# jmduarte/gnn-fpga

Measured on AMD Instinct MI355X. Metric: edges/sec (EdgeNet+NodeNet fwd) on 100k-edge TrackML graphs; % HBM roofline, higher is better.
Workload: dtype f32; 1 GPU; c3 synthetic TrackML ACTS graphs: 256 graphs/launch/GPU x (10k hits, 100k segments), F=3, D=8, 3 MP iterations + final edge pass, index form resident in HBM; graphs_per_gpu=256, hits_per_graph=10000, segments_per_graph=100000

## Files before the change

### gnn-fpga_amd/csrc/sell_pipeline.hip

```cpp
#include "common.h"

#include <cstdlib>
#include <type_traits>
#include <utility>

namespace {
using namespace gnn;

constexpr int SLICE = 16;
constexpr int DESC = 8;

template <int F, int D>
struct TL {
    static constexpr int d4 = D / 4, C = F + D;
    static constexpr int a4(int x) { return (x + 3) & ~3; }
    static constexpr int o_w2 = 0;
    static constexpr int o_in = a4(o_w2 + d4);
    static constexpr int in_sz = d4 + F * d4;
    static constexpr int o_4 = a4(o_in + in_sz);
    static constexpr int w4_sz = d4 + D * d4;
    static constexpr int o_m = a4(o_4 + w4_sz);
    static constexpr int m_sz = d4 + C * d4;
    static constexpr int m_st = a4(m_sz);
    static constexpr int o_b2 = o_m + 5 * m_st;
// ... 1430 lines not shown
    __device__ __forceinline__ void second(float *f) const { f[0] = bf_lo(w.z); f[1] = bf_hi(w.z); f[2] = bf_lo(w.w); f[3] = bf_hi(w.w); }
};
template <> struct PieceW<1> {
    unsigned w;
    __device__ __forceinline__ void load(const void *a) { w = *reinterpret_cast<const unsigned *>(a); }
    __device__ __forceinline__ void first(float *f) const { f[0] = bf_lo(w); }
    __device__ __forceinline__ void second(float *f) const { f[0] = bf_hi(w); }
};
template <> struct PieceW<2> {
    uint2 w;
    __device__ __forceinline__ void load(const void *a) { w = *reinterpret_cast<const uint2 *>(a); }
    __device__ __forceinline__ void first(float *f) const { f[0] = bf_lo(w.x); f[1] = bf_hi(w.x); }
    __device__ __forceinline__ void second(float *f) const { f[0] = bf_lo(w.y); f[1] = bf_hi(w.y); }
};
template <int DL> struct PieceX;
template <> struct PieceX<4> {
    float4 a, b;
    __device__ __forceinline__ void load(const void *p)
    {
        a = reinterpret_cast<const float4 *>(p)[0];
        b = reinterpret_cast<const float4 *>(p)[16];
    }
    __device__ __forceinline__ void first(float *f) const { f[0] = a.x; f[1] = a.y; f[2] = a.z; f[3] = a.w; }
    __device__ __forceinline__ void second(float *f) const { f[0] = b.x; f[1] = b.y; f[2] = b.z; f[3] = b.w; }
};
template <> struct PieceX<1> {
    float2 a;
    __device__ __forceinline__ void load(const void *p) { a = *reinterpret_cast<const float2 *>(p); }
    __device__ __forceinline__ void first(float *f) const { f[0] = a.x; }
    __device__ __forceinline__ void second(float *f) const { f[0] = a.y; }
};
template <> struct PieceX<2> {
    float4 a;
    __device__ __forceinline__ void load(const void *p) { a = *reinterpret_cast<const float4 *>(p); }
    __device__ __forceinline__ void first(float *f) const { f[0] = a.x; f[1] = a.y; }
    __device__ __forceinline__ void second(float *f) const { f[0] = a.z; f[1] = a.w; }
};

template <int D, bool EX = false>
struct RecW {
    static constexpr int DL = D / 16;
    static constexpr unsigned row_bytes = (EX ? 8 : 4) * D;
    static constexpr unsigned piece_bytes = row_halves<D, EX>() ? 4 * DL : (EX ? 8 : 4) * DL;
    std::conditional_t<EX, PieceX<DL>, PieceW<DL>> r[4];
    __device__ __forceinline__ void read(int cur, const void *__restrict__ REC, unsigned lane_off)
    {
        const int nb[4] = {quad_bcast_i<0>(cur), quad_bcast_i<1>(cur), quad_bcast_i<2>(cur), quad_bcast_i<3>(cur)};
#pragma unroll
        for (int j = 0; j < 4; ++j)
            r[j].load(reinterpret_cast<const char *>(REC) + ((unsigned)nb[j] * row_bytes + lane_off));
    }
};

template <int D, bool XP, bool EX = false>
__device__ __forceinline__ void score_w(const RecW<D, EX> &g, const float *own, const float *w2, float b2, int p,
                                        float *acc)
{
    constexpr int DL = D / 16;
    static_assert(DL == 1 || DL % 2 == 0, "one dimension per lane, or dimension pairs");
    const f2_t one2 = {1.0f, 1.0f};
    float part[4];
#pragma unroll
    for (int j = 0; j < 4; ++j) {
        float P[DL];
        g.r[j].first(P);
        if constexpr (DL == 1) {
            const float a = XP ? fmaf(P[0], own[0], 1.0f) : __builtin_amdgcn_exp2f(P[0] + own[0]) + 1.0f;
            part[j] = w2[0] * __builtin_amdgcn_rcpf(a);
        } else {
            f2_t s2 = {0.0f, 0.0f};
#pragma unroll
            for (int i = 0; i + 1 < DL; i += 2) {
                const f2_t pj = {P[i], P[i + 1]}, o2 = {own[i], own[i + 1]};
                f2_t a;
                if constexpr (XP) {
                    a = pj * o2 + one2;
                } else {
                    const f2_t z = pj + o2;
                    a = f2_t{__builtin_amdgcn_exp2f(z.x), __builtin_amdgcn_exp2f(z.y)} + one2;
                }
                const f2_t r = {__builtin_amdgcn_rcpf(a.x), __builtin_amdgcn_rcpf(a.y)};
                s2 = f2_t{w2[i], w2[i + 1]} * r + s2;
            }
            part[j] = s2.x + s2.y;
        }
    }
    const int q = p & 3;
    const bool odd = q & 1, hi = q & 2;
    const float s0 = odd ? part[0] : part[1], s1 = odd ? part[2] : part[3];
    const float k0 = odd ? part[1] : part[0], k1 = odd ? part[3] : part[2];
    const float t0 = k0 + dpp<0xB1>(s0), t1 = k1 + dpp<0xB1>(s1);
    const float give = hi ? t0 : t1, keep = hi ? t1 : t0;
    float mine = keep + dpp<0x4E>(give);
    mine += dpp_row<0x124>(mine);
    mine += dpp_row<0x128>(mine);
    const float e = r_f(mine + b2);
    const float e4[4] = {quad_bcast_f<0>(e), quad_bcast_f<1>(e), quad_bcast_f<2>(e), quad_bcast_f<3>(e)};
#pragma unroll
    for (int j = 0; j < 4; ++j) {
        float R[DL];
        g.r[j].second(R);
        if constexpr (DL == 1) {
            acc[0] = fmaf(R[0], e4[j], acc[0]);
        } else {
            const f2_t e2 = {e4[j], e4[j]};
#pragma unroll
            for (int i = 0; i + 1 < DL; i += 2) {
                const f2_t a2 = f2_t{R[i], R[i + 1]} * e2 + f2_t{acc[i], acc[i + 1]};
                acc[i] = a2.x;
                acc[i + 1] = a2.y;
            }
        }
    }
}

template <int D, bool XP, bool EX = false>
__device__ __forceinline__ void sweep_w(const int32_t *__restrict__ lst, int i16, int len, int null_idx,
                                        const void *__restrict__ REC, int p, const float *own, const float *w2,
                                        float b2, float *acc)
{
    if (len <= 0) return;
    constexpr int DL = D / 16;
    const int ng = (len + 3) >> 2;
    const unsigned lane_off = RecW<D, EX>::piece_bytes * (unsigned)p;
    const unsigned st_off = (unsigned)((SLICE * (p & 3) + i16) * 4);
    auto index_of = [&](int c) {
        const int cur = *reinterpret_cast<const int32_t *>(reinterpret_cast<const char *>(lst) +
                                                             ((unsigned)(c * 4 * SLICE * 4) + st_off));
        return 4 * c + (p & 3) < len ? cur : null_idx;
    };
    RecW<D, EX> a, b;
    int ia = index_of(0), ib = ng > 1 ? index_of(1) : 0;
    a.read(ia, REC, lane_off);
    for (int c = 0; c < ng; c += 2) {
        if (c + 1 < ng) b.read(ib, REC, lane_off);
        if (c + 2 < ng) ia = index_of(c + 2);
        score_w<D, XP, EX>(a, own, w2, b2, p, acc);
        if (c + 1 < ng) {
            if (c + 2 < ng) a.read(ia, REC, lane_off);
            if (c + 3 < ng) ib = index_of(c + 3);
            score_w<D, XP, EX>(b, own, w2, b2, p, acc);
        }
    }
}

template <int D, bool EX>
__device__ __forceinline__ void load_own_w(const unsigned *__restrict__ REC, int64_t n, int p, float *out)
{
    constexpr int DL = D / 16;
    if constexpr (row_halves<D, EX>()) {
        load_vec<DL>(reinterpret_cast<const float *>(REC) + n * 2 * D + DL * p, out);
    } else {
        constexpr int WPR = EX ? 2 * D : D, WPL = EX ? 2 * DL : DL;
        std::conditional_t<EX, PieceX<DL>, PieceW<DL>> w;
        w.load(REC + n * WPR + WPL * p);
        w.first(out);
    }
}

template <int F, int D, bool LAST, bool XP, bool EX = false>
__global__ __launch_bounds__(1024, (D == 16 ? 8 : 4)) void k_iter_w(
    const float *__restrict__ X, const float *__restrict__ table, const unsigned *__restrict__ t16,
    const int32_t *__restrict__ tiles, const int32_t *__restrict__ in_off, const int32_t *__restrict__ in_nbr,
    const int32_t *__restrict__ out_off, const int32_t *__restrict__ out_nbr, const unsigned *__restrict__ PR,
    const unsigned *__restrict__ QS, float *__restrict__ U, float *__restrict__ PRn, float *__restrict__ QSn,
    float *__restrict__ Pc, float *__restrict__ Qc, int64_t n_pad, int tiles_per_xcd, int n_tiles, int wmax)
{
    using L = TL<F, D>;
    using B = std::conditional_t<EX, BX<F, D>, BL<F, D>>;
    static_assert(D % 16 == 0, "16 lanes x D / 16 dims per hit, matrix-core tail");
    extern __shared__ __attribute__((aligned(16))) float smem[];
    int *grp = reinterpret_cast<int *>(smem + B::template lds_words<LAST>() + (EX ? 12 : 8) * 16 * B::tr_stride);
    unsigned *tb = reinterpret_cast<unsigned *>(smem);
    {
        constexpr int n1 = B::NT1 * B::KS1 * (EX ? 64 : 256), nm = B::template tm_words<LAST>();
        for (int i = threadIdx.x; i < n1; i += 1024) tb[i] = t16[B::o_t4 + i];
        for (int i = threadIdx.x; i < nm; i += 1024) tb[n1 + i] = t16[(LAST ? B::o_tml : B::o_tmn) + i];
        for (int i = threadIdx.x; i < D; i += 1024) tb[n1 + nm + i] = t16[B::o_b4 + i];
        for (int i = threadIdx.x; i < (LAST ? 2 : 5) * D; i += 1024)
            tb[n1 + nm + D + i] = t16[(LAST ? B::o_bml : B::o_bmn) + i];
    }
    const int lane = threadIdx.x & 63, wv = threadIdx.x >> 6;
    const int hs = lane >> 4, p = lane & 15;
    const int team = wv >> 2, mem = wv & 3;
    float *scratch = smem + B::template lds_words<LAST>();
    constexpr int DL = D / 16;
    float w2[DL];
#pragma unroll
    for (int i = 0; i < DL; ++i) w2[i] = table[(p >> 2) * L::stride + L::o_w2 + DL * (p & 3) + i];
    const float b2 = table[L::o_b2];
    const int xcd = blockIdx.x & 7, local = blockIdx.x >> 3, per_xcd = gridDim.x >> 3;
    const int t_begin = xcd * tiles_per_xcd;
    const int t_end = t_begin + tiles_per_xcd < n_tiles ? t_begin + tiles_per_xcd : n_tiles;
    __syncthreads();
    if (t_begin >= t_end) return;
    int buf = 0, rot = 0;
    for (int t = t_begin; t < t_end;) {
        if (wv == 0) {
            const int tt = t + lane;
            const bool in = tt < t_end;
            const int32_t *d = tiles + (int64_t)(in ? tt : t) * DESC;
            const int s1 = d[1];
            int ilo = in && d[3] > 0 ? d[2] : 0x7FFFFFFF, ihi = in && d[3] > 0 ? d[2] + d[3] : -1;
            int olo = in && d[5] > 0 ? d[4] : 0x7FFFFFFF, ohi = in && d[5] > 0 ? d[4] + d[5] : -1;
#pragma unroll
            for (int o = 1; o < 64; o <<= 1) {
                const int a = __shfl_up(ilo, o, 64), b = __shfl_up(ihi, o, 64);
                const int c = __shfl_up(olo, o, 64), e = __shfl_up(ohi, o, 64);
                if (lane >= o) {
                    ilo = a < ilo ? a : ilo; ihi = b > ihi ? b : ihi;
                    olo = c < olo ? c : olo; ohi = e > ohi ? e : ohi;
                }
            }
            const bool ok = in && (lane == 0 || ((int64_t)ihi - ilo <= wmax && (int64_t)ohi - olo <= wmax));
            const unsigned long long m = ~__ballot(ok);
            const int cnt = m ? __builtin_ctzll(m) : 64;
            const int send = __shfl(s1, cnt - 1, 64);
            if (lane == 0) { grp[0] = d[0]; grp[1] = send; grp[2] = t + cnt; }
        }
        __syncthreads();
        const int sg0 = grp[0], sg1 = grp[1];
        t = grp[2];
        __syncthreads();
        const int nq = (sg1 - sg0 + 3) >> 2;
        const int q0 = (((local - rot) % per_xcd) + per_xcd) % per_xcd;
        rot = (rot + nq) % per_xcd;
        const int x0 = sg0;
        constexpr bool SPLIT = EX && D >= 64;
        for (int q = q0; SPLIT && x0 + 4 * q < sg1; q += per_xcd) {
            const int sl = x0 + 4 * q + team;
            if (sl < sg0 || sl >= sg1) continue;
            const int ib = __builtin_amdgcn_readfirstlane(in_off[sl]);
            const int il = (__builtin_amdgcn_readfirstlane(in_off[sl + 1]) - ib) >> 4;
            if (il <= 0) continue;
            const int i16 = 4 * mem + hs;
            const int64_t n = (int64_t)sl * SLICE + i16;
            float acc[DL], ownQ[DL];
            load_vec<DL>(U + n * D + DL * p, acc);
            load_own_w<D, EX>(QS, n, p, ownQ);
#ifndef GNN_ABLATE_W_SWEEP
            sweep_w<D, XP, EX>(in_nbr + ib, i16, il, (int)n_pad, PR, p, ownQ, w2, b2, acc);
#endif
            store_vec<DL>(U + n * D + DL * p, acc);
        }
        for (int q = q0; x0 + 4 * q < sg1; q += per_xcd, buf ^= 1) {
            const int sl = x0 + 4 * q + team;
            const bool on = sl >= sg0 && sl < sg1;
            float *tr = scratch + (buf * 4 + team) * 16 * B::tr_stride;
            if (on) {
                const int ob = __builtin_amdgcn_readfirstlane(out_off[sl]);
                const int ol = (__builtin_amdgcn_readfirstlane(out_off[sl + 1]) - ob) >> 4;
                const int i16 = 4 * mem + hs;
                const int64_t n = (int64_t)sl * SLICE + i16;
                float acc[DL], ownP[DL];
                load_vec<DL>(U + n * D + DL * p, acc);
                if constexpr (!SPLIT) {
                    const int ib = __builtin_amdgcn_readfirstlane(in_off[sl]);
                    const int il = (__builtin_amdgcn_readfirstlane(in_off[sl + 1]) - ib) >> 4;
                    float ownQ[DL];
                    load_own_w<D, EX>(QS, n, p, ownQ);
                    load_own_w<D, EX>(PR, n, p, ownP);
                    sweep_w<D, XP, EX>(in_nbr + ib, i16, il, (int)n_pad, PR, p, ownQ, w2, b2, acc);
                } else {
                    load_own_w<D, EX>(PR, n, p, ownP);
                }
#ifndef GNN_ABLATE_W_SWEEP
                sweep_w<D, XP, EX>(out_nbr + ob, i16, ol, (int)n_pad, QS, p, ownP, w2, b2, acc);
#endif
#pragma unroll
                for (int i = 0; i < DL; ++i) acc[i] = tanh_f(acc[i]);
                store_vec<DL>(tr + i16 * B::tr_stride + DL * p, acc);
                if (p < F) tr[i16 * B::tr_stride + D + p] = X[n * F + p];
            }
            __syncthreads();
            if constexpr (EX) {
                float *th = scratch + (8 + team) * 16 * B::tr_stride;
#ifndef GNN_ABLATE_W_TAIL
                if (on) mfma_hidden_x<F, D, LAST>(smem, tr, th, lane, mem);
#endif
                __syncthreads();
#ifndef GNN_ABLATE_W_TAIL
                if (on)
                    mfma_tail_scratch_x<F, D, LAST, XP>(smem, tr, th, lane, (int64_t)sl * SLICE, PRn, QSn, U, Pc, Qc, mem, 4);
#endif
            } else if (on) {
                mfma_tail_scratch<F, D, LAST, XP>(tb, tr, lane, (int64_t)sl * SLICE, PRn, QSn, U, Pc, Qc, mem, 4);
            }
        }
    }
}

template <int F, int D, bool LAST, bool XP, bool EX = true>
__global__ __launch_bounds__(1024, (D == 16 ? 8 : 4)) void k_iter_wx(
    const float *__restrict__ X, const float *__restrict__ table, const unsigned *__restrict__ t16,
    const int32_t *__restrict__ tiles, const int32_t *__restrict__ in_off, const int32_t *__restrict__ in_nbr,
    const int32_t *__restrict__ out_off, const int32_t *__restrict__ out_nbr, const unsigned *__restrict__ PR,
    const unsigned *__restrict__ QS, float *__restrict__ U, float *__restrict__ PRn, float *__restrict__ QSn,
    float *__restrict__ Pc, float *__restrict__ Qc, int64_t n_pad, int tiles_per_xcd, int n_tiles, int wmax)
{
    using L = TL<F, D>;
    using B = std::conditional_t<EX, BX<F, D>, BL<F, D>>;
    constexpr int DL = D / 16, NSLOT = 12, NSW = 12, NMX = 4, NTEAM = NSW / 4;
    constexpr int n1 = B::NT1 * B::KS1 * (EX ? 64 : 256), nm = B::template tm_words<LAST>();
    typedef float f4v __attribute__((ext_vector_type(4)));
    extern __shared__ __attribute__((aligned(16))) float smem[];
    float *ring = smem + B::template lds_words<LAST>();
    int *sync = reinterpret_cast<int *>(ring + NSLOT * 16 * B::tr_stride);
    int *prod = sync, *cons = sync + NSLOT, *meta = sync + 2 * NSLOT, *fin = sync + 3 * NSLOT, *pha = fin + 1;
    {
        unsigned *tb = reinterpret_cast<unsigned *>(smem);
        for (int i = threadIdx.x; i < n1; i += 1024) tb[i] = t16[B::o_t4 + i];
        for (int i = threadIdx.x; i < nm; i += 1024) tb[n1 + i] = t16[(LAST ? B::o_tml : B::o_tmn) + i];
        for (int i = threadIdx.x; i < D; i += 1024) tb[n1 + nm + i] = t16[B::o_b4 + i];
        for (int i = threadIdx.x; i < (LAST ? 2 : 5) * D; i += 1024)
            tb[n1 + nm + D + i] = t16[(LAST ? B::o_bml : B::o_bmn) + i];
        if (threadIdx.x < 3 * NSLOT + 2) sync[threadIdx.x] = 0;
    }
    __syncthreads();
    const int lane = threadIdx.x & 63, wv = __builtin_amdgcn_readfirstlane(threadIdx.x >> 6);
    auto ld = [](const int *w) { return __hip_atomic_load(w, __ATOMIC_RELAXED, __HIP_MEMORY_SCOPE_WORKGROUP); };
// ... 193 lines not shown
{
    if constexpr (D == 8) return MT<F, D>::total;
    else return 0;
}

template <int F, int D>
__device__ __forceinline__ float mt_entry(const gnn_params_t &p, int i, bool last)
{
    using M = MT<F, D>;
    constexpr int C = F + D;
    if (i < 64) {
        const int row = i & 15, g = i >> 4;
        return (row < 8 && g < F && g < 4) ? p.Win[row * F + g] : 0.0f;
    }
    if (i < M::o_w4) {
        const int j = i - M::o_t, T = j / M::t_sz, st = (j % M::t_sz) >> 6, row = j & 15, g = (j >> 4) & 3;
        const int k = M::slot_k(st, g);
        if (k < 0) return 0.0f;
        if (last) {
            if (T > 0) return 0.0f;
            return kTwoLog2e * p.W1[(row & 7) * 2 * C + (row >> 3) * C + k];
        }
        if (T == 2) return row < 8 ? p.W3[row * 3 * C + 2 * C + k] : 0.0f;
        const int c = row >> 2, w = row & 3, d = 2 * c + (w & 1);
        return (w < 2) ? kTwoLog2e * p.W1[d * 2 * C + T * C + k] : p.W3[d * 3 * C + T * C + k];
    }
    if (i < M::o_b) {
        const int j = i - M::o_w4, st = j >> 6, row = j & 15, g = (j >> 4) & 3;
        return row < 8 ? p.W4[row * D + 2 * g + st] : 0.0f;
    }
    const int j = i - M::o_b, which = j >> 4, row = j & 15;
    switch (which) {
    case 0: return row < 8 ? p.bin[row] : 0.0f;
    case 1:
        if (last) return row < 8 ? kTwoLog2e * p.b1[row] : 0.0f;
        return (row & 3) < 2 ? kTwoLog2e * p.b1[2 * (row >> 2) + (row & 1)] : 0.0f;
    case 2: return 0.0f;
    case 3: return (!last && row < 8) ? p.b3[row] : 0.0f;
    default: return row < 8 ? p.b4[row] : 0.0f;
    }
}

template <int F, int D, bool LAST, bool XP, bool FIRST>
__global__ __launch_bounds__(1024) void k_iter2(
    const float *__restrict__ X, const float *__restrict__ table, gnn_params_t p,
    float *__restrict__ table_out,
    const int32_t *__restrict__ tiles, const int32_t *__restrict__ in_off,
    const int32_t *__restrict__ in_off16, const int32_t *__restrict__ in_nbr16,
    const int32_t *__restrict__ out_off, const int32_t *__restrict__ out_off16,
    const int32_t *__restrict__ out_nbr16, const int32_t *__restrict__ sched_a,
    const int32_t *__restrict__ sched_b, const float *__restrict__ PR,
    const float *__restrict__ QS, float *__restrict__ U, float *__restrict__ PRn,
    float *__restrict__ QSn, float *__restrict__ Pc, float *__restrict__ Qc, int64_t n_pad,
    int n_tiles, int capA, int capB, int xbuf_floats)
{
    using L = TL<F, D>;
    constexpr int d4 = L::d4, NT = 1024, NWV = NT / 64, NC = 3;
    extern __shared__ __attribute__((aligned(16))) float smem[];
    float *lds = smem, *bufA = smem + L::total, *bufB = bufA + (int64_t)capA * 2 * D;
    float *xbuf = bufB + (int64_t)capB * 2 * D;
    const int tid = threadIdx.x, lane = tid & 63, q = lane & 3, i16 = lane >> 2;
    const int wv = __builtin_amdgcn_readfirstlane(tid >> 6);
    if constexpr (FIRST) {
        for (int idx = tid; idx < L::total; idx += NT) {
            const float v = table_entry<F, D>(p, idx);
            lds[idx] = v;
            if (blockIdx.x == 0) table_out[idx] = v;
        }
        if (blockIdx.x == 0)
            write_null_rows<F, D, XP>(p, PRn, const_cast<float *>(PR), QSn, const_cast<float *>(QS),
                                      U, Pc, Qc, n_pad);
    } else {
        stage4<NT>(table, lds, L::total / 4);
    }
    float *mt = xbuf + (FIRST ? xbuf_floats : 0);
    if constexpr (D == 8)
        for (int i = tid; i < MT<F, D>::total; i += NT) mt[i] = mt_entry<F, D>(p, i, LAST);
    int tile = (gridDim.x & 7) ? (int)blockIdx.x
                               : (int)((blockIdx.x & 7) * (gridDim.x >> 3) + (blockIdx.x >> 3));
    if (tile >= n_tiles) return;

    struct Desc { int s_begin, s_end, in_lo, in_cnt, out_lo, out_cnt, sbase; };
    auto load_desc = [&](int t) {
        const int32_t *td = tiles + (int64_t)t * DESC;
        Desc d;
        d.s_begin = td[0]; d.s_end = td[1]; d.in_lo = td[2]; d.in_cnt = td[3];
        d.out_lo = td[4]; d.out_cnt = td[5]; d.sbase = td[7];
        return d;
    };
    auto slice_a = [&](const Desc &d, int r) { return sched_a[d.sbase + r * NWV + wv]; };

    auto stage_issue = [&](const float *src, float *buf, int nrec) {
        const int pieces = (nrec * 2 * D + 255) / 256;
        unsigned lb = (unsigned)lane * 16u;
        asm volatile("" : "+v"(lb));
        for (int c = wv; c < pieces; c += NWV)
            __builtin_amdgcn_global_load_lds(
                (const __attribute__((address_space(1))) void *)(
                    reinterpret_cast<const char *>(src + (int64_t)c * 256) + lb),
                (__attribute__((address_space(3))) void *)(buf + c * 256), 16, 0, 0);
    };
    auto put_null = [&](float *buf, int nrec, auto which) {
        constexpr int M = decltype(which)::value;
        const int pieces = (nrec * 2 * D + 255) / 256;
        if (wv == (pieces > 0 ? (pieces - 1) % NWV : 0) && lane < 4) {
            int l = lane;
            asm volatile("" : "+v"(l));
#pragma unroll
            for (int i = 0; i < d4; ++i) {
                float v = (M == 0) ? lds[l * L::stride + L::o_m + i] : 0.0f, z = 0.0f;
                if (XP) v = (M == 0) ? __builtin_amdgcn_exp2f(v) : 1.0f;
                asm volatile("" : "+v"(v), "+v"(z));
                buf[nrec * 2 * D + l * 2 * d4 + i] = v;
                buf[nrec * 2 * D + l * 2 * d4 + d4 + i] = z;
            }
        }
    };
    using WinA = std::integral_constant<int, 0>;
    using WinB = std::integral_constant<int, 1>;
    auto stage_commit = [&](float *buf, int nrec, auto which) {
        a_wait_all();
        put_null(buf, nrec, which);
    };

    auto x_image = [&](float *buf, int cap) { return buf + cap * 2 * D - (cap * F + 63) / 64 * 64; };
    auto xstage_issue = [&](int lo, int cnt, float *buf, int cap) {
        const int pieces = (cnt * F + 63) / 64;
        float *xb = x_image(buf, cap);
        unsigned lb = (unsigned)lane * 4u;
        asm volatile("" : "+v"(lb));
        for (int c = wv; c < pieces; c += NWV)
            __builtin_amdgcn_global_load_lds(
                (const __attribute__((address_space(1))) void *)(
                    reinterpret_cast<const char *>(X + (int64_t)lo * F + c * 64) + lb),
                (__attribute__((address_space(3))) void *)(xb + c * 64), 4, 0, 0);
    };
    auto h0_of = [&](const float *wl, const float *x, float *hn) {
// ... 355 lines not shown
                        } else if (T < 2) {
                            if constexpr (XP) {
                                c.x = __builtin_amdgcn_exp2f(c.x);
                                c.y = __builtin_amdgcn_exp2f(c.y);
                            }
                            *reinterpret_cast<f4v *>((T == 0 ? PRn : QSn) + n * 2 * D + 4 * g) = c;
                        } else if (g < 2) {
                            *reinterpret_cast<f4v *>(U + n * D + 4 * g) = c;
                        }
                    }
                }
            } else if (slice >= 0) {
                int woff = q * L::stride;
                asm volatile("" : "+v"(woff));
                const float *wl = lds + woff;
                float ql[d4], qa[D], hl[d4], hn[D];
#pragma unroll
                for (int i = 0; i < d4; ++i) ql[i] = tanh_f(acc[i]);
                quad_allgather<d4>(ql, qa);
                role_gemv<d4, D, 0>(wl + L::o_4, qa, qa, hl);
#pragma unroll
                for (int i = 0; i < d4; ++i) hl[i] = tanh_f(hl[i]);
                quad_allgather<d4>(hl, hn);
                const int64_t n0 = (int64_t)__builtin_amdgcn_readfirstlane(slice) * SLICE;
                auto at = [](float *base, unsigned off) {
                    return reinterpret_cast<float *>(reinterpret_cast<char *>(base) + off);
                };
                if constexpr (LAST)
                    emit_to<F, D, LAST, XP>(wl, hn, xv, at(Pc + n0 * D, lo_vec), at(Qc + n0 * D, lo_vec), nullptr);
                else
                    emit_to<F, D, LAST, XP>(wl, hn, xv, at(PRn + n0 * 2 * D, lo_rec), at(QSn + n0 * 2 * D, lo_rec),
                                            at(U + n0 * D, lo_vec));
            }
        };
        for (int r = 0; r + 1 < rounds; ++r) roundB(r, std::false_type{});
        roundB(rounds - 1, std::true_type{});
        if (tnext >= n_tiles) break;
        if constexpr (FIRST)
            compute_window(bufA, dn.in_cnt, capA, WinA{});
        else
            stage_commit(bufA, dn.in_cnt, WinA{});
        if (slice_a(dn, 0) >= 0) arriveA(a_cur);
        tile = tnext;
        d = dn;
    }
}

template <int F, int D, bool XP>
__global__ __launch_bounds__((Cfg<F, D>::NT)) void k_edge(
    const int32_t *__restrict__ chunks, const int32_t *__restrict__ src,
    const int32_t *__restrict__ dst, const int32_t *__restrict__ sd16,
    const float *__restrict__ Pc, const float *__restrict__ Qc,
    const float *__restrict__ table, float *__restrict__ e, int64_t n_pad, int chunks_per_xcd,
    int n_chunks)
{
    using G = Cfg<F, D>;
    const float *__restrict__ W2 = table + TL<F, D>::o_flat;
    constexpr int NT = G::NT;
    extern __shared__ __attribute__((aligned(16))) float win[];
    const int chunk = (blockIdx.x & 7) * chunks_per_xcd + (blockIdx.x >> 3);
    if (chunk >= n_chunks) return;
    const int32_t *cd = chunks + (int64_t)chunk * DESC;
    const int e0 = cd[0], e1 = cd[1], s_lo = cd[2], s_cnt = cd[3], d_lo = cd[4], d_cnt = cd[5],
              mode = cd[6];
    float *winA = win, *winB = win + (s_cnt + 1) * D;
    if (G::ed_rec > 0 && mode) {
        stage4<NT>(Pc + (int64_t)s_lo * D, winA, s_cnt * D / 4);
        stage4<NT>(Pc + n_pad * D, winA + s_cnt * D, D / 4);
        stage4<NT>(Qc + (int64_t)d_lo * D, winB, d_cnt * D / 4);
        stage4<NT>(Qc + n_pad * D, winB + d_cnt * D, D / 4);
        __syncthreads();
    }
    const float b2 = W2[D];
    auto score = [&](const float *p, const float *qq) {
        float acc = b2;
#pragma unroll
        for (int k = 0; k < D; ++k)
            acc = fmaf(W2[k], XP ? __builtin_amdgcn_rcpf(fmaf(p[k], qq[k], 1.0f)) : r_f(p[k] + qq[k]), acc);
        return r_f(acc);
    };
    if (G::ed_rec > 0 && mode) {
        constexpr int B8 = 8;
        for (int j0 = e0 + (int)threadIdx.x; j0 < e1; j0 += B8 * NT) {
            unsigned w[B8];
#pragma unroll
            for (int u = 0; u < B8; ++u) w[u] = (j0 + u * NT < e1) ? (unsigned)sd16[j0 + u * NT] : 0u;
#pragma unroll
            for (int u = 0; u < B8; ++u) {
                if (j0 + u * NT < e1) {
                    float p[D], qq[D];
                    load_vec<D>(winA + (w[u] & 0xFFFFu) * D, p);
                    load_vec<D>(winB + (w[u] >> 16) * D, qq);
                    e[j0 + u * NT] = score(p, qq);
                }
            }
        }
    } else {
        for (int j = e0 + (int)threadIdx.x; j < e1; j += NT) {
            float p[D], qq[D];
            const int s = src[j], d = dst[j];
            load_vec<D>(Pc + (int64_t)s * D, p);
            load_vec<D>(Qc + (int64_t)d * D, qq);
            e[j] = score(p, qq);
        }
    }
}

template <int F, int D, bool XP>
__global__ __launch_bounds__(256) void k_edge_tw(const int32_t *__restrict__ src, const int32_t *__restrict__ dst,
                                                 const float *__restrict__ Pc, const float *__restrict__ Qc,
                                                 const float *__restrict__ table, float *__restrict__ e, int64_t n_pad,
                                                 int64_t n_segments)
{
    const float *__restrict__ W2 = table + TL<F, D>::o_flat;
// ... 120 lines not shown
    int family;
    bool fuse_first;
    int edge;
    bool pack;
    int64_t it_lds;
    int64_t it2_lds;
    int64_t capA, capB;
    int64_t ed_lds;
    int wmax;
};

template <int F, int D, bool XP>
Route choose_route(const gnn_plan_t *pl, const gnn_params_t *p, int n_iters, const Switches &sw, bool training = false)
{
    using L = TL<F, D>;
    using G = Cfg<F, D>;
    const int64_t Np = pl->n_pad, nt = pl->n_tiles;
    Route r{};
    r.supported = !training || (D <= 16 && !G::wide16);
    if (!r.supported) return r;
    constexpr bool can_bf = D % 32 == 0 && F <= 8;
    const bool bf = !training && can_bf && (p->flags & GNN_FLAG_BF16_MLP) && n_iters > 0 && Np > 0 &&
                    (uint64_t)(Np + 2) * D * 4 < (1ull << 32);
    constexpr bool can_ex = D % 16 == 0 && F <= 4;
    const bool ex = !training && can_ex && !bf && n_iters > 0 && Np > 0 && (uint64_t)(Np + 2) * D * 8 < (1ull << 32) &&
                    !sw.no_wide_exact;
    r.rec = bf ? GNN_REC_BF16 : ex ? GNN_REC_EXACT : GNN_REC_FP32;
    r.pack = Np == 0 || G::pack_first || ex;
    r.edge = (!training && G::ed_rec == 0 && D % 16 == 0) ? GNN_EDGE_K_EDGE_W : GNN_EDGE_K_EDGE;
    r.ed_lds = (int64_t)(((G::ed_rec > 0 ? pl->edge_lds_rows : 0) * D + 4) * sizeof(float));
    r.input = GNN_INPUT_NONE;
    r.family = GNN_FAMILY_K_ITER;
    if (Np == 0) return r;
    r.it_lds = (int64_t)((L::total + (G::it_rec > 0 ? pl->iter_lds_records : 0) * 2 * D + 4) * sizeof(float));
    bool use2 = false;
    if constexpr (G::iter2) {
        const int64_t rpp = 128 / D;
        r.capA = (pl->iter_lds_in + rpp - 1) / rpp * rpp + rpp;
        r.capB = (pl->iter_lds_out + rpp - 1) / rpp * rpp + rpp;
        r.it2_lds = (int64_t)((L::total + (r.capA + r.capB) * 2 * D + 4 + mt_total<F, D>()) * sizeof(float));
        use2 = !training && !sw.no_iter2 && nt > 0 && pl->n_lds_tiles == nt && pl->in_nbr16 && pl->out_nbr16 &&
               pl->in_off16 && pl->out_off16 && pl->sched_a && pl->sched_b && r.it2_lds <= G::lds_bytes;
        r.fuse_first = G::fuse_first && XP && use2 && n_iters >= 2 && !sw.no_fuse_first;
    }
    const bool lockstep = sw.wide_lockstep || (Np < kRoleSplitMinHits && !sw.wide_roles);
    r.family = (bf || ex) ? (lockstep ? GNN_FAMILY_K_ITER_W : GNN_FAMILY_K_ITER_WX) : use2 ? GNN_FAMILY_K_ITER2 : GNN_FAMILY_K_ITER;
    r.wmax = bf ? wide_window_records(4 * D) : ex ? wide_window_records(8 * D) : 0;
    r.input = r.fuse_first ? GNN_INPUT_NONE
              : (bf && G::pack_first) ? GNN_INPUT_K_INPUT4_BF
              : ex ? GNN_INPUT_K_INPUT4_X : GNN_INPUT_K_INPUT4;
    return r;
}

template <typename Fn>
int with_flag(bool flag, Fn &&fn)
{
    return flag ? fn(std::true_type{}) : fn(std::false_type{});
}

template <auto Kernel>
void lds_opt_in(int bytes)
{
    static DevOnce once;
    if (once.need())
        (void)hipFuncSetAttribute(reinterpret_cast<const void *>(Kernel), hipFuncAttributeMaxDynamicSharedMemorySize, bytes);
}

struct TrainArgs {
    const int32_t *seg_ptr, *tw_src, *tw_dst;
    float *e_all, *H_all, *Q_all;
    int ldh;
};

struct Run {
    const gnn_plan_t *pl;
    const gnn_params_t *p;
    Route r;
    Ws w;
    hipStream_t s;
    int ablate;
    float *PR, *PRn, *QS, *QSn;
};

template <int F, int D, bool XP, bool TR>
int launch_input(const Run &c, bool last, float *H0, int ldh)
{
    using G = Cfg<F, D>;
    const int64_t Np = c.pl->n_pad;
    const Ws &w = c.w;
    if (c.r.input == GNN_INPUT_K_INPUT4_BF) {
        if constexpr (D % 32 == 0 && F <= 8) {
            using B = BL<F, D>;
            const size_t lds_in = (size_t)(B::template tm_words<false>() + 5 * D + 4 * 16 * B::tr_stride) * 4;
            lds_opt_in<&k_input4_bf<F, D, false, XP>>(G::lds_bytes);
            const int64_t g_need = (Np * 4 + 255) / 256;
            GNN_LAUNCH_SH("k_input4", (k_input4_bf<F, D, false, XP>), (unsigned)(g_need < 512 ? g_need : 512), 256,
                          lds_in, c.s, c.pl->X, w.table, w.t16, c.PR, c.QS, w.U, w.Pc, w.Qc, Np);
        }
    } else if (c.r.input == GNN_INPUT_K_INPUT4_X) {
        if constexpr (D % 16 == 0 && F <= 4) {
            using B = BX<F, D>;
            const size_t lds_in = (size_t)(B::template tm_words<false>() + 5 * D + 16 * 16 * B::tr_stride) * 4;
            lds_opt_in<&k_input4_x<F, D, false, XP>>(G::lds_bytes);
            const int64_t g_need = (Np * 4 + 1023) / 1024;
            const int64_t g_cap = device_cus();
            GNN_LAUNCH_SH("k_input4", (k_input4_x<F, D, false, XP>), (unsigned)(g_need < g_cap ? g_need : g_cap), 1024,
                          lds_in, c.s, c.pl->X, w.table, reinterpret_cast<const float *>(w.t16), c.PR, c.QS, w.U, w.Pc,
                          w.Qc, Np);
        }
    } else if (c.r.input == GNN_INPUT_K_INPUT4) {
        const int64_t g_need = (Np * 4 + 255) / 256;
        const unsigned g = (unsigned)(g_need < 4096 ? g_need : 4096);
        return with_flag(last, [&](auto last_c) {
            GNN_LAUNCH("k_input4", (k_input4<F, D, decltype(last_c)::value, XP, TR>), g, 256, c.s, c.pl->X, *c.p, w.table,
                       c.PR, c.QS, c.PRn, c.QSn, w.U, w.Pc, w.Qc, Np, H0, ldh);
            return 0;
        });
    }
    return 0;
}

template <int F, int D, bool XP, bool TR>
int launch_iter(const Run &c, bool last, const TrainOut &tro)
{
    using G = Cfg<F, D>;
    const gnn_plan_t *pl = c.pl;
    const Ws &w = c.w;
    const int nt = (int)pl->n_tiles, tpx = (nt + 7) / 8;
    return with_flag(last, [&](auto last_c) {
        constexpr bool LAST = decltype(last_c)::value;
        lds_opt_in<&k_iter<F, D, LAST, XP, TR>>(G::lds_bytes);
        GNN_LAUNCH_SH("k_iter", (k_iter<F, D, LAST, XP, TR>), 8 * tpx, G::NT, (size_t)c.r.it_lds, c.s, pl->X, w.table,
                      pl->tiles, pl->in_off, pl->in_nbr, pl->out_off, pl->out_nbr, c.PR, c.QS, w.U, c.PRn, c.QSn, w.Pc,
                      w.Qc, pl->n_pad, tpx, nt, c.ablate, tro);
        return 0;
    });
}

template <int F, int D, bool XP>
int launch_iter2(const Run &c, bool first, bool last)
{
    using G = Cfg<F, D>;
    const gnn_plan_t *pl = c.pl;
    const Ws &w = c.w;
    const int nt = (int)pl->n_tiles, n_cu = device_cus();
    const int grid = nt < n_cu ? nt : n_cu;
    const auto launch = [&](auto last_c, auto first_c) {
        constexpr bool LAST = decltype(last_c)::value, FIRST = decltype(first_c)::value;
        lds_opt_in<&k_iter2<F, D, LAST, XP, FIRST>>(G::lds_bytes);
        GNN_LAUNCH_SH("k_iter2", (k_iter2<F, D, LAST, XP, FIRST>), grid, 1024, (size_t)c.r.it2_lds, c.s, pl->X, w.table,
                      *c.p, w.table, pl->tiles, pl->in_off, pl->in_off16, pl->in_nbr16, pl->out_off, pl->out_off16,
                      pl->out_nbr16, pl->sched_a, pl->sched_b, c.PR, c.QS, w.U, c.PRn, c.QSn, w.Pc, w.Qc, pl->n_pad, nt,
                      (int)c.r.capA, (int)c.r.capB, 0);
        return 0;
    };
    if constexpr (XP && G::fuse_first)
        if (first) return launch(std::false_type{}, std::true_type{});
    return with_flag(last, [&](auto last_c) { return launch(last_c, std::false_type{}); });
}

template <int F, int D, bool XP, bool EX>
int launch_wide(const Run &c, bool last)
{
    using G = Cfg<F, D>;
    using B = std::conditional_t<EX, BX<F, D>, BL<F, D>>;
    const gnn_plan_t *pl = c.pl;
    const Ws &w = c.w;
    const int nt = (int)pl->n_tiles, tpx = (nt + 7) / 8;
    const int ncu = device_cus() * (EX && D == 16 ? 2 : 1);
    const unsigned wgs = (unsigned)(((nt < ncu ? nt : ncu) + 7) / 8 * 8);
    const unsigned *PRh = reinterpret_cast<const unsigned *>(c.PR), *QSh = reinterpret_cast<const unsigned *>(c.QS);
    return with_flag(last, [&](auto last_c) {
        constexpr bool LAST = decltype(last_c)::value;
        if (c.r.family == GNN_FAMILY_K_ITER_WX) {
            const size_t ringw = (size_t)12 * 16 * B::tr_stride + 40;
            lds_opt_in<&k_iter_wx<F, D, LAST, XP, EX>>(G::lds_bytes);
            GNN_LAUNCH_SH("k_iter_wx", (k_iter_wx<F, D, LAST, XP, EX>), wgs, 1024,
                          (B::template lds_words<LAST>() + ringw) * 4, c.s, pl->X, w.table, w.t16, pl->tiles, pl->in_off,
                          pl->in_nbr, pl->out_off, pl->out_nbr, PRh, QSh, w.U, c.PRn, c.QSn, w.Pc, w.Qc, pl->n_pad, tpx,
                          nt, c.r.wmax);
        } else {
            const size_t trw = (size_t)(EX ? 2 * 4 + 4 : 2 * 4) * 16 * B::tr_stride + 4;
            lds_opt_in<&k_iter_w<F, D, LAST, XP, EX>>(G::lds_bytes);
            GNN_LAUNCH_SH("k_iter_w", (k_iter_w<F, D, LAST, XP, EX>), wgs, 1024,
                          (B::template lds_words<LAST>() + trw) * 4, c.s, pl->X, w.table, w.t16, pl->tiles, pl->in_off,
                          pl->in_nbr, pl->out_off, pl->out_nbr, PRh, QSh, w.U, c.PRn, c.QSn, w.Pc, w.Qc, pl->n_pad, tpx,
                          nt, c.r.wmax);
        }
        return 0;
    });
}

template <int F, int D, bool XP>
int launch_edge(const Run &c, float *e_out)
{
    using G = Cfg<F, D>;
    const gnn_plan_t *pl = c.pl;
    const Ws &w = c.w;
    const int64_t E = pl->n_segments;
    lds_opt_in<&k_edge<F, D, XP>>(G::lds_bytes);
    if (c.r.edge == GNN_EDGE_K_EDGE_W) {
        if constexpr (G::ed_rec == 0 && D % 16 == 0) {
            const int64_t waves = (E + 15) / 16;
            int64_t wg = (waves + 3) / 4;
            const int64_t cap = (int64_t)device_cus() * 8;
            wg = wg < cap ? wg : cap;
            GNN_LAUNCH("k_edge", (k_edge_w<F, D, XP>), (unsigned)((wg + 7) / 8 * 8), 256, c.s, pl->src, pl->dst, w.Pc,
                       w.Qc, w.table, e_out, E);
        }
    } else {
        const int nc = (int)pl->n_chunks, cpx = (nc + 7) / 8;
        GNN_LAUNCH_SH("k_edge", (k_edge<F, D, XP>), 8 * cpx, G::NT, (size_t)c.r.ed_lds, c.s, pl->chunks, pl->src, pl->dst,
                      pl->sd16, w.Pc, w.Qc, w.table, e_out, pl->n_pad, cpx, nc);
    }
    return 0;
}

template <int F, int D, bool XP, bool TR>
int forward_t(const gnn_plan_t *pl, const gnn_params_t *p, int n_iters, const Switches &sw, const TrainArgs &tr,
              float *e_out, char *ws, hipStream_t s)
{
    using G = Cfg<F, D>;
    if constexpr (TR && (D > 16 || G::wide16)) {
        return fail(GNN_ERR_UNSUPPORTED, "no fused training forward for input_dim=%d hidden_dim=%d", F, D);
    } else {
        const int64_t Np = pl->n_pad, E = pl->n_segments;
        const Ws w = carve<F, D>(ws, Np);
        Run c{pl, p, choose_route<F, D, XP>(pl, p, n_iters, sw, TR), w, s, TR ? 0 : sw.ablate, w.PRa, w.PRb, w.QSa, w.QSb};
        if constexpr (D % 32 == 0 && F <= 8)
            if (c.r.rec == GNN_REC_BF16)
                GNN_LAUNCH("k_pack16", (k_pack16<F, D>), 64, 256, s, *p, w.t16, w.PRa, w.PRb, w.QSa, w.QSb, Np, XP ? 1 : 0);
        if (c.r.pack)
            GNN_LAUNCH("k_pack", (k_pack<F, D, XP>), (TL<F, D>::total + 255) / 256, 256, s, *p, w.table, w.PRa, w.PRb,
                       w.QSa, w.QSb, w.U, w.Pc, w.Qc, Np);
        if constexpr (D % 16 == 0 && F <= 4)
            if (c.r.rec == GNN_REC_EXACT)
                GNN_LAUNCH("k_pack32", (k_pack32<F, D>), 64, 256, s, *p, reinterpret_cast<float *>(w.t16), w.PRa, w.PRb,
                           w.QSa, w.QSb, Np, XP ? 1 : 0);
        if (Np > 0) {
            if (int rc = launch_input<F, D, XP, TR>(c, n_iters == 0, tr.H_all, tr.ldh)) return rc;
            for (int t = 0; t < n_iters; ++t) {
                const bool last = t + 1 == n_iters;
                int rc = 0;
                if (c.r.family == GNN_FAMILY_K_ITER) {
                    TrainOut tro{};
                    if constexpr (TR)
                        tro = TrainOut{tr.seg_ptr, tr.e_all + (size_t)t * E, tr.Q_all + (size_t)t * Np * D,
                                       tr.H_all + (size_t)(t + 1) * Np * tr.ldh, tr.ldh};
                    rc = launch_iter<F, D, XP, TR>(c, last, tro);
                } else if constexpr (!TR) {
                    if (c.r.family == GNN_FAMILY_K_ITER2) {
                        if constexpr (G::iter2) rc = launch_iter2<F, D, XP>(c, t == 0 && c.r.fuse_first, last);
                    } else if (c.r.rec == GNN_REC_BF16) {
                        if constexpr (D % 32 == 0 && F <= 8) rc = launch_wide<F, D, XP, false>(c, last);
                    } else {
                        if constexpr (D % 16 == 0 && F <= 4) rc = launch_wide<F, D, XP, true>(c, last);
                    }
                }
                if (rc) return rc;
                std::swap(c.PR, c.PRn);
                std::swap(c.QS, c.QSn);
            }
        }
        if (E > 0 && (!TR || e_out))
            if (int rc = launch_edge<F, D, XP>(c, e_out)) return rc;
        if constexpr (TR)
            if (E > 0 && tr.tw_src)
                GNN_LAUNCH("k_edge_tw", (k_edge_tw<F, D, XP>), grid_for(E), 256, s, tr.tw_src, tr.tw_dst, w.Pc, w.Qc,
                           w.table, tr.e_all + (size_t)n_iters * E, Np, E);
        return 0;
    }
}

#ifdef GNN_QUICK
#ifndef GNN_QUICK_F
#define GNN_QUICK_F 3
#endif
#ifndef GNN_QUICK_D
#define GNN_QUICK_D 8
#endif
#define SELL_FOR_EACH_SHAPE(X_) X_(GNN_QUICK_F, GNN_QUICK_D)
#else
#define SELL_FOR_EACH_SHAPE(X_)                                                          \
    X_(2, 4) X_(2, 8) X_(2, 16) X_(2, 32) X_(3, 4) X_(3, 8) X_(3, 16) X_(3, 32) X_(3, 64) \
    X_(11, 4) X_(11, 8) X_(11, 16)
#endif

template <bool TR>
int forward_any(const gnn_plan_t *pl, const gnn_params_t *p, int n_iters, const TrainArgs &tr, float *e_out, void *ws,
                size_t ws_bytes, hipStream_t s)
{
    ProfChain chain_;
    const size_t need = sell_workspace_bytes(pl->n_pad, pl->n_segments, p->F, p->D);
    if (need == 0) return fail(GNN_ERR_UNSUPPORTED, "no fused kernel for input_dim=%d hidden_dim=%d", p->F, p->D);
    if (int rc = check_workspace(ws, ws_bytes, need)) return rc;
    const Switches sw = read_switches();
#define X_(F_, D_)                                                                                            \
    if (p->F == F_ && p->D == D_)                                                                            \
        return (p->flags & GNN_FLAG_EXP_PRODUCT) ? forward_t<F_, D_, true, TR>(pl, p, n_iters, sw, tr, e_out, align_ws(ws), s) \
                                                 : forward_t<F_, D_, false, TR>(pl, p, n_iters, sw, tr, e_out, align_ws(ws), s);
    SELL_FOR_EACH_SHAPE(X_)
#undef X_
    return fail(GNN_ERR_UNSUPPORTED, "unreachable");
}

}

namespace gnn {

int sell_shape_supported(int F, int D)
{
#define X_(F_, D_) if (F == F_ && D == D_) return 1;
    SELL_FOR_EACH_SHAPE(X_)
#undef X_
    return 0;
}

int sell_limits(int F, int D, int32_t *out4)
// ... 59 lines not shown
```

Baseline: 30.67 billion edges/s.

## Trim tail neighbour loads in wide sweep and alternate tile walk direction

The wide-record sweep now loads and scores only the valid neighbours in the final group of four. Before, it padded that group with null-index rows and still scored them. Separately, the k_iter2 iterations and the final edge kernel now walk tiles or chunks in reverse on alternate passes. The aim is for the start of each pass to hit data the previous pass left in cache. Trimming adds divergent branches and extra template instantiations, and the reversed order relies on L2/MALL reuse that may not hold across launches.

```diff
diff --git a/gnn-fpga_amd/csrc/sell_pipeline.hip b/gnn-fpga_amd/csrc/sell_pipeline.hip
--- a/gnn-fpga_amd/csrc/sell_pipeline.hip
+++ b/gnn-fpga_amd/csrc/sell_pipeline.hip
@@ -1506,16 +1506,16 @@
     }
 };
 
-template <int D, bool XP, bool EX = false>
+template <int D, bool XP, bool EX = false, int REM = 4>
 __device__ __forceinline__ void score_w(const RecW<D, EX> &g, const float *own, const float *w2, float b2, int p,
                                         float *acc)
 {
     constexpr int DL = D / 16;
     static_assert(DL == 1 || DL % 2 == 0, "one dimension per lane, or dimension pairs");
     const f2_t one2 = {1.0f, 1.0f};
-    float part[4];
-#pragma unroll
-    for (int j = 0; j < 4; ++j) {
+    float part[4] = {0.0f, 0.0f, 0.0f, 0.0f};
+#pragma unroll
+    for (int j = 0; j < REM; ++j) {
         float P[DL];
         g.r[j].first(P);
         if constexpr (DL == 1) {
@@ -1551,7 +1551,7 @@
     const float e = r_f(mine + b2);
     const float e4[4] = {quad_bcast_f<0>(e), quad_bcast_f<1>(e), quad_bcast_f<2>(e), quad_bcast_f<3>(e)};
 #pragma unroll
-    for (int j = 0; j < 4; ++j) {
+    for (int j = 0; j < REM; ++j) {
         float R[DL];
         g.r[j].second(R);
         if constexpr (DL == 1) {
@@ -1568,7 +1568,7 @@
     }
 }
 
-template <int D, bool XP, bool EX = false>
+template <int D, bool XP, bool EX = false, bool TRIM = true>
 __device__ __forceinline__ void sweep_w(const int32_t *__restrict__ lst, int i16, int len, int null_idx,
                                         const void *__restrict__ REC, int p, const float *own, const float *w2,
                                         float b2, float *acc)
@@ -1584,16 +1584,50 @@
         return 4 * c + (p & 3) < len ? cur : null_idx;
     };
     RecW<D, EX> a, b;
+#ifdef GNN_NO_TRIM
+    constexpr bool trim = false;
+#else
+    constexpr bool trim = TRIM;
+#endif
     int ia = index_of(0), ib = ng > 1 ? index_of(1) : 0;
-    a.read(ia, REC, lane_off);
-    for (int c = 0; c < ng; c += 2) {
-        if (c + 1 < ng) b.read(ib, REC, lane_off);
-        if (c + 2 < ng) ia = index_of(c + 2);
-        score_w<D, XP, EX>(a, own, w2, b2, p, acc);
-        if (c + 1 < ng) {
-            if (c + 2 < ng) a.read(ia, REC, lane_off);
-            if (c + 3 < ng) ib = index_of(c + 3);
-            score_w<D, XP, EX>(b, own, w2, b2, p, acc);
+    if constexpr (!trim) {
+        a.read(ia, REC, lane_off);
+        for (int c = 0; c < ng; c += 2) {
+            if (c + 1 < ng) b.read(ib, REC, lane_off);
+            if (c + 2 < ng) ia = index_of(c + 2);
+            score_w<D, XP, EX>(a, own, w2, b2, p, acc);
+            if (c + 1 < ng) {
+                if (c + 2 < ng) a.read(ia, REC, lane_off);
+                if (c + 3 < ng) ib = index_of(c + 3);
+                score_w<D, XP, EX>(b, own, w2, b2, p, acc);
+            }
+        }
+    } else {
+        auto read_n = [&](RecW<D, EX> &g, int idx, int n) {
+            const int nb[4] = {quad_bcast_i<0>(idx), quad_bcast_i<1>(idx), quad_bcast_i<2>(idx), quad_bcast_i<3>(idx)};
+            const char *base = reinterpret_cast<const char *>(REC);
+            constexpr unsigned rb = RecW<D, EX>::row_bytes;
+            g.r[0].load(base + ((unsigned)nb[0] * rb + lane_off));
+            if (n > 1) g.r[1].load(base + ((unsigned)nb[1] * rb + lane_off));
+            if (n > 2) g.r[2].load(base + ((unsigned)nb[2] * rb + lane_off));
+            if (n > 3) g.r[3].load(base + ((unsigned)nb[3] * rb + lane_off));
+        };
+        auto score_n = [&](const RecW<D, EX> &g, int n) {
+            if (n >= 4) score_w<D, XP, EX>(g, own, w2, b2, p, acc);
+            else if (n == 3) score_w<D, XP, EX, 3>(g, own, w2, b2, p, acc);
+            else if (n == 2) score_w<D, XP, EX, 2>(g, own, w2, b2, p, acc);
+            else score_w<D, XP, EX, 1>(g, own, w2, b2, p, acc);
+        };
+        read_n(a, ia, len);
+        for (int c = 0; c < ng; c += 2) {
+            if (c + 1 < ng) read_n(b, ib, len - 4 * (c + 1));
+            if (c + 2 < ng) ia = index_of(c + 2);
+            score_n(a, len - 4 * c);
+            if (c + 1 < ng) {
+                if (c + 2 < ng) read_n(a, ia, len - 4 * (c + 2));
+                if (c + 3 < ng) ib = index_of(c + 3);
+                score_n(b, len - 4 * (c + 1));
+            }
         }
     }
 }
@@ -1620,6 +1654,7 @@
     const unsigned *__restrict__ QS, float *__restrict__ U, float *__restrict__ PRn, float *__restrict__ QSn,
     float *__restrict__ Pc, float *__restrict__ Qc, int64_t n_pad, int tiles_per_xcd, int n_tiles, int wmax)
 {
+    constexpr bool TRIMW = !(EX && D == 64);
     using L = TL<F, D>;
     using B = std::conditional_t<EX, BX<F, D>, BL<F, D>>;
     static_assert(D % 16 == 0, "16 lanes x D / 16 dims per hit, matrix-core tail");
@@ -1693,7 +1728,7 @@
             load_vec<DL>(U + n * D + DL * p, acc);
             load_own_w<D, EX>(QS, n, p, ownQ);
 #ifndef GNN_ABLATE_W_SWEEP
-            sweep_w<D, XP, EX>(in_nbr + ib, i16, il, (int)n_pad, PR, p, ownQ, w2, b2, acc);
+            sweep_w<D, XP, EX, TRIMW>(in_nbr + ib, i16, il, (int)n_pad, PR, p, ownQ, w2, b2, acc);
 #endif
             store_vec<DL>(U + n * D + DL * p, acc);
         }
@@ -1714,12 +1749,12 @@
                     float ownQ[DL];
                     load_own_w<D, EX>(QS, n, p, ownQ);
                     load_own_w<D, EX>(PR, n, p, ownP);
-                    sweep_w<D, XP, EX>(in_nbr + ib, i16, il, (int)n_pad, PR, p, ownQ, w2, b2, acc);
+                    sweep_w<D, XP, EX, TRIMW>(in_nbr + ib, i16, il, (int)n_pad, PR, p, ownQ, w2, b2, acc);
                 } else {
                     load_own_w<D, EX>(PR, n, p, ownP);
                 }
 #ifndef GNN_ABLATE_W_SWEEP
-                sweep_w<D, XP, EX>(out_nbr + ob, i16, ol, (int)n_pad, QS, p, ownP, w2, b2, acc);
+                sweep_w<D, XP, EX, TRIMW>(out_nbr + ob, i16, ol, (int)n_pad, QS, p, ownP, w2, b2, acc);
 #endif
 #pragma unroll
                 for (int i = 0; i < DL; ++i) acc[i] = tanh_f(acc[i]);
@@ -2019,7 +2054,7 @@
     const int32_t *__restrict__ sched_b, const float *__restrict__ PR,
     const float *__restrict__ QS, float *__restrict__ U, float *__restrict__ PRn,
     float *__restrict__ QSn, float *__restrict__ Pc, float *__restrict__ Qc, int64_t n_pad,
-    int n_tiles, int capA, int capB, int xbuf_floats)
+    int n_tiles, int capA, int capB, int xbuf_floats, int backward)
 {
     using L = TL<F, D>;
     constexpr int d4 = L::d4, NT = 1024, NWV = NT / 64, NC = 3;
@@ -2049,7 +2084,7 @@
 
     struct Desc { int s_begin, s_end, in_lo, in_cnt, out_lo, out_cnt, sbase; };
     auto load_desc = [&](int t) {
-        const int32_t *td = tiles + (int64_t)t * DESC;
+        const int32_t *td = tiles + (int64_t)(backward ? n_tiles - 1 - t : t) * DESC;
         Desc d;
         d.s_begin = td[0]; d.s_end = td[1]; d.in_lo = td[2]; d.in_cnt = td[3];
         d.out_lo = td[4]; d.out_cnt = td[5]; d.sbase = td[7];
@@ -2511,14 +2546,15 @@
     const int32_t *__restrict__ dst, const int32_t *__restrict__ sd16,
     const float *__restrict__ Pc, const float *__restrict__ Qc,
     const float *__restrict__ table, float *__restrict__ e, int64_t n_pad, int chunks_per_xcd,
-    int n_chunks)
+    int n_chunks, int backward)
 {
     using G = Cfg<F, D>;
     const float *__restrict__ W2 = table + TL<F, D>::o_flat;
     constexpr int NT = G::NT;
     extern __shared__ __attribute__((aligned(16))) float win[];
-    const int chunk = (blockIdx.x & 7) * chunks_per_xcd + (blockIdx.x >> 3);
-    if (chunk >= n_chunks) return;
+    const int pos = (blockIdx.x & 7) * chunks_per_xcd + (blockIdx.x >> 3);
+    if (pos >= n_chunks) return;
+    const int chunk = backward ? n_chunks - 1 - pos : pos;
     const int32_t *cd = chunks + (int64_t)chunk * DESC;
     const int e0 = cd[0], e1 = cd[1], s_lo = cd[2], s_cnt = cd[3], d_lo = cd[4], d_cnt = cd[5],
               mode = cd[6];
@@ -2745,6 +2781,25 @@
     return r;
 }
 
+inline bool walks_backward(const Route &r, int t)
+{
+#ifdef GNN_FORWARD_WALK
+    (void)r; (void)t;
+    return false;
+#else
+    return r.family == GNN_FAMILY_K_ITER2 && (t & 1);
+#endif
+}
+inline bool edge_walks_backward(const Route &r, int n_iters)
+{
+#ifdef GNN_FORWARD_WALK
+    (void)r; (void)n_iters;
+    return false;
+#else
+    return r.family == GNN_FAMILY_K_ITER2 && n_iters > 0 && !walks_backward(r, n_iters - 1);
+#endif
+}
+
 template <typename Fn>
 int with_flag(bool flag, Fn &&fn)
 {
@@ -2831,7 +2886,7 @@
 }
 
 template <int F, int D, bool XP>
-int launch_iter2(const Run &c, bool first, bool last)
+int launch_iter2(const Run &c, bool first, bool last, bool backward)
 {
     using G = Cfg<F, D>;
     const gnn_plan_t *pl = c.pl;
@@ -2844,7 +2899,7 @@
         GNN_LAUNCH_SH("k_iter2", (k_iter2<F, D, LAST, XP, FIRST>), grid, 1024, (size_t)c.r.it2_lds, c.s, pl->X, w.table,
                       *c.p, w.table, pl->tiles, pl->in_off, pl->in_off16, pl->in_nbr16, pl->out_off, pl->out_off16,
                       pl->out_nbr16, pl->sched_a, pl->sched_b, c.PR, c.QS, w.U, c.PRn, c.QSn, w.Pc, w.Qc, pl->n_pad, nt,
-                      (int)c.r.capA, (int)c.r.capB, 0);
+                      (int)c.r.capA, (int)c.r.capB, 0, backward ? 1 : 0);
         return 0;
     };
     if constexpr (XP && G::fuse_first)
@@ -2885,7 +2940,7 @@
 }
 
 template <int F, int D, bool XP>
-int launch_edge(const Run &c, float *e_out)
+int launch_edge(const Run &c, float *e_out, bool backward)
 {
     using G = Cfg<F, D>;
     const gnn_plan_t *pl = c.pl;
@@ -2904,7 +2959,7 @@
     } else {
         const int nc = (int)pl->n_chunks, cpx = (nc + 7) / 8;
         GNN_LAUNCH_SH("k_edge", (k_edge<F, D, XP>), 8 * cpx, G::NT, (size_t)c.r.ed_lds, c.s, pl->chunks, pl->src, pl->dst,
-                      pl->sd16, w.Pc, w.Qc, w.table, e_out, pl->n_pad, cpx, nc);
+                      pl->sd16, w.Pc, w.Qc, w.table, e_out, pl->n_pad, cpx, nc, backward ? 1 : 0);
     }
     return 0;
 }
@@ -2943,7 +2998,8 @@
                     rc = launch_iter<F, D, XP, TR>(c, last, tro);
                 } else if constexpr (!TR) {
                     if (c.r.family == GNN_FAMILY_K_ITER2) {
-                        if constexpr (G::iter2) rc = launch_iter2<F, D, XP>(c, t == 0 && c.r.fuse_first, last);
+                        if constexpr (G::iter2)
+                            rc = launch_iter2<F, D, XP>(c, t == 0 && c.r.fuse_first, last, walks_backward(c.r, t));
                     } else if (c.r.rec == GNN_REC_BF16) {
                         if constexpr (D % 32 == 0 && F <= 8) rc = launch_wide<F, D, XP, false>(c, last);
                     } else {
@@ -2956,7 +3012,7 @@
             }
         }
         if (E > 0 && (!TR || e_out))
-            if (int rc = launch_edge<F, D, XP>(c, e_out)) return rc;
+            if (int rc = launch_edge<F, D, XP>(c, e_out, edge_walks_backward(c.r, n_iters))) return rc;
         if constexpr (TR)
             if (E > 0 && tr.tw_src)
                 GNN_LAUNCH("k_edge_tw", (k_edge_tw<F, D, XP>), grid_for(E), 256, s, tr.tw_src, tr.tw_dst, w.Pc, w.Qc,
```

Measured after the change: 31.12 billion edges/s (median of 6 runs). 1.5% higher.
